# microsoft/fadtk

Measured on AMD Instinct MI355X. Metric: FAD scores/sec + cov-GEMM TFLOP/s (% MFMA peak), N=100k D=512, higher is better.
Workload: dtype f16 in, f16 MFMA with f32 accumulate over <= 8192-row runs, f64 across runs (moments); split-f16 MFMA iterations (f32 accumulate) + exact int8-MFMA products (int32 accumulate) + f64 correction (Frechet)

## Files before the change

### fadtk_amd/csrc/frechet.hip

```cpp
#include "frechet_internal.h"
#include "ns_mean.h"
#include "ns_fast.h"
#include "ns_fast_big.h"
#include "ns_fast_res.h"

#include <algorithm>
#include <atomic>
#include <cmath>
#include <type_traits>

namespace fad {

Pool& thread_pool(int device) {
    static thread_local PerThreadDevice<Pool> set;
    return set.get(device);
}
Workspace* free_slot(int device) {
    Pool& p = thread_pool(device);
    for (Workspace& w : p.slot)
        if (!w.busy) { w.pool = &p; return &w; }
    return nullptr;
}

SongKnobs SongKnobs::from_env() {
// ... 582 lines not shown
    int k = 1, upto = resident ? 1 : 9;
    for (;;) {
        for (; k < upto; ++k) {
            const int cur = k & 1;
            nsf::SplitArgs g = split_args();
            g.A[0] = Z[cur]; g.B[0] = Y[cur]; g.C[0] = T; g.alpha = -0.5f; g.beta_eye = 1.5f; g.gamma = 1.0f;
            g.partials = partials; g.skip = &s32_0->done; g.k = k;
            if (big) FAD_TRY(fast_split_big(d, nsf::SP_T, g, st, (unsigned)B, device));
            else fast_split(d, nsf::SP_T, g, st, (unsigned)B);
            g = split_args();
            g.A[0] = Y[cur]; g.B[0] = T; g.C[0] = Y[cur ^ 1]; g.A[1] = T; g.B[1] = Z[cur]; g.C[1] = Z[cur ^ 1];
            g.skip = &s32_0->upd_skip[k & 1];
            g.k = k; g.max_low = kMaxLow; g.nslots = big ? fast_big_t_slots(d, (unsigned)B) : nb * nb; g.chk_partials = partials; g.thr_pred = pred_threshold(ws.pool, d);
            if (big) FAD_TRY(fast_split_big(d, nsf::SP_U, g, st, (unsigned)B, device));
            else fast_split(d, nsf::SP_U, g, st, (unsigned)B);
        }
        if (!res_full) {
            nsf::DigArgs dg;
            memset(&dg, 0, sizeof(dg));
            dg.d = d; dg.gen = gen; dg.hA = hdr_b; dg.hB = reinterpret_cast<nsf::MatHdr*>(at(L.hdr)); dg.pstride = (int64_t)L.stride; dg.s32 = s32_0;
            dg.Y[0] = Y[0]; dg.Y[1] = Y[1]; dg.dig[0] = digY[0]; dg.dig[1] = digY[1]; dg.dig_t[0] = digYt[0]; dg.dig_t[1] = digYt[1];
            hipLaunchKernelGGL(nsf::nsf_digitize, dim3((unsigned)((dd / 16 + 255) / 256), 2, (unsigned)B), dim3(256), 0, st, dg);
        }
        if (!res_full) {
            nsf::I8Args a;
            memset(&a, 0, sizeof(a));
            a.Adig = digY[0]; a.Bdig = digYt[0]; a.Adig_alt = digY[1]; a.Bdig_alt = digYt[1]; a.sel = &s32_0->final_iter;
            a.d = d; a.gen = gen; a.hA = hdr_b; a.hB = reinterpret_cast<nsf::MatHdr*>(at(L.hdr)); a.pstride = (int64_t)L.stride; a.hstride = (int64_t)hs;
            a.skip = &s32_0->skip_corr; a.stats = h_stats; a.st = st0; a.A64in = A64;
            a.Y[0] = Y[0]; a.Y[1] = Y[1]; a.Z[0] = Z[0]; a.Z[1] = Z[1]; a.s32 = s32_0; a.host_words = h_words; a.host_vals = h_vals;
            for (int64_t b = 0; b < B; ++b) reinterpret_cast<int*>(reinterpret_cast<char*>(h_words) + b * hs)[12] = 0;
            if (big && d >= 256) FAD_TRY(fast_i8_big(d, nsf::I8_G, a, st, (unsigned)B, device));
            else fast_i8(d, nsf::I8_G, a, st, (unsigned)B);
        }
        FAD_HIP_TRY(hipGetLastError());
        FAD_HIP_TRY(hipStreamSynchronize(st));
        bool pending = false;
        for (int64_t b = 0; b < B; ++b) {
            if (settled[b]) continue;
            const int* hw = reinterpret_cast<const int*>(reinterpret_cast<const char*>(h_words) + b * hs);
            const double* hv = reinterpret_cast<const double*>(reinterpret_cast<const char*>(h_vals) + b * hs);
            const double* hx = reinterpret_cast<const double*>(reinterpret_cast<const char*>(h_stats) + b * hs);
            if (hw[12] != gen) return set_error(FAD_ERR_HIP, "the correction kernel of the batched fast chain left no result for song %lld", (long long)b);
            MixedResult r;
            fast_decide_one(hw, hv, hx, nb, &r);
            if (r.status == 0 && k < kMaxLow && !resident) { pending = true; continue; }
            settled[b] = 1;
            if (r.status == 1) { ok[b] = 1; tr_sqrt[b] = std::sqrt(r.c) * r.tr_scaled; }
            if (trace)
                fprintf(stderr, "[fad fast songs] song %lld: status %d iters %d decided_at %d res %.3e est %.3e tr %.6e c %.3e (words bad %d done %d ok %d failed %d skipped %d)\n",
                        (long long)b, r.status, r.iters, r.decided_at, r.res, r.est, r.tr_scaled, r.c, hw[0], hw[1], hw[5], hw[6], hw[11]);
            if (trace && b == 0) {
                fprintf(stderr, "[fad fast songs] song 0 residuals:");
                for (int q = 1; q < 16 && q <= r.iters; ++q) fprintf(stderr, " %.3e", hv[4 + q]);
                fprintf(stderr, "\n");
            }
        }
        if (!pending) break;
        upto = kMaxLow;
    }
    return FAD_OK;
}


struct PairBlock {
    size_t hdrA, hdrB, st, s32, partials, stats, A64, P, Y[2], Z[2], T, digA, digB, digY[2], digYt[2], mus, covs, Rv, Pv, Ev, stride;
};
static PairBlock pair_block(int d) {
    const size_t dd = (size_t)d * d, nb = (size_t)d / 32;
    PairBlock b; size_t o = 0;
    auto take = [&](size_t bytes) { const size_t at = o; o += (bytes + 255) & ~(size_t)255; return at; };
    b.hdrA = take(sizeof(nsf::MatHdr)); b.hdrB = take(sizeof(nsf::MatHdr)); b.st = take(sizeof(NsState)); b.s32 = take(sizeof(Ns32State));
    b.partials = take(nb * nb * sizeof(double)); b.stats = take(nsf::kTileStats * nb * nb * sizeof(double));
    b.A64 = take(8 * dd); b.P = take(8 * dd);
    b.Y[0] = take(8 * dd); b.Y[1] = take(8 * dd); b.Z[0] = take(8 * dd); b.Z[1] = take(8 * dd); b.T = take(8 * dd);
    b.digA = take(6 * dd); b.digB = take(6 * dd);
    b.digY[0] = take(6 * dd); b.digYt[0] = take(6 * dd); b.digY[1] = take(6 * dd); b.digYt[1] = take(6 * dd);
    b.mus = take(2 * (size_t)d * sizeof(double)); b.covs = take(2 * dd * sizeof(double));
    b.Rv = take(8 * dd); b.Pv = take(8 * dd); b.Ev = take(8 * dd);
    b.stride = o;
    return b;
}

static int pairs_verify_enqueue(Workspace& ws, int d, int B, hipStream_t st) {
    const size_t dd = (size_t)d * d;
    const PairBlock L = pair_block(d);
    const size_t hs = song_host_stride(d);
    char* blk = static_cast<char*>(ws.fast_pairs.p);
    char* hpin = static_cast<char*>(ws.fast_pairs_pin);
    auto at = [&](size_t off) { return blk + off; };
    auto mat = [&](size_t off) { nsf::SplitMat m; m.a = reinterpret_cast<uint4*>(at(off)); m.at = reinterpret_cast<uint4*>(at(off + 4 * dd)); return m; };
    nsf::SplitArgs g;
    memset(&g, 0, sizeof(g));
    g.d = d; g.gen = ws.multi.gen; g.hA = reinterpret_cast<nsf::MatHdr*>(at(L.hdrA)); g.hB = reinterpret_cast<nsf::MatHdr*>(at(L.hdrB));
    g.pstride = (int64_t)L.stride; g.astride = (int64_t)L.stride;
    g.st = reinterpret_cast<NsState*>(at(L.st)); g.s32 = reinterpret_cast<Ns32State*>(at(L.s32));
    const nsf::SplitMat Y[2] = {mat(L.Y[0]), mat(L.Y[1])}, Z[2] = {mat(L.Z[0]), mat(L.Z[1])};
    const int nb = d / 32;
    int* h_words = reinterpret_cast<int*>(hpin + (nsf::kHostVals + (size_t)(nsf::kTileStats + 2) * nb * nb) * sizeof(double));
    double* h_vstats = reinterpret_cast<double*>(hpin + host_vstats_off(d));
    for (int b = 0; b < B; ++b) reinterpret_cast<int*>(reinterpret_cast<char*>(h_words) + (size_t)b * hs)[13] = 0;
    fast_verify_launch(d, (unsigned)B, g, Y, Z, mat(L.Rv), mat(L.Pv), mat(L.Ev), g.s32, h_vstats, h_words, (int64_t)hs, st);
    FAD_HIP_TRY(hipGetLastError());
    FAD_HIP_TRY(hipEventRecord(ws.done_ev, st));
    return FAD_OK;
}

static int pairs_enqueue(Workspace& ws, int d, int B, const fad_moments_t* const* h1, const fad_moments_t* const* h2, int ddof,
                         int mean_dtype, hipStream_t st) {
    const size_t dd = (size_t)d * d;
    const int nb = d / 32;
    constexpr int kPairsBigMin = 3;
    const bool big = B >= kPairsBigMin && d >= 256;
    const bool wide = wide_enabled(ws.pool);
    const int max_low = wide ? kMaxLowWide : kMaxLow;
    const int device = ws.job.device;
    const PairBlock L = pair_block(d);
    const size_t hs = song_host_stride(d);
    void* const before = ws.fast_pairs.p;
    FAD_TRY(ws.fast_pairs.reserve((size_t)(B > 16 ? kMaxMultiPairs : B > 8 ? 16 : B > 4 ? 8 : 4) * L.stride + 256));
    if (!ws.fast_pairs_pin || ws.fast_pairs_pin_cap < (size_t)B * hs) {
        if (ws.fast_pairs_pin) (void)hipHostFree(ws.fast_pairs_pin);
        ws.fast_pairs_pin = nullptr; ws.fast_pairs_pin_cap = 0;
        FAD_HIP_TRY(hipHostMalloc(&ws.fast_pairs_pin, (size_t)kMaxMultiPairs * hs + 4096, hipHostMallocDefault));
        ws.fast_pairs_pin_cap = (size_t)kMaxMultiPairs * hs + 4096;
    }
    char* blk = static_cast<char*>(ws.fast_pairs.p);
    char* hpin = static_cast<char*>(ws.fast_pairs_pin);
    double* h_vals = reinterpret_cast<double*>(hpin);
    double* h_stats = h_vals + nsf::kHostVals;
    int* h_words = reinterpret_cast<int*>(h_stats + (size_t)(nsf::kTileStats + 2) * nb * nb);
    auto at = [&](size_t off) { return blk + off; };
    auto mat = [&](size_t off) { nsf::SplitMat m; m.a = reinterpret_cast<uint4*>(at(off)); m.at = reinterpret_cast<uint4*>(at(off + 4 * dd)); return m; };
    const int gen = ++ws.fast_gen;
    if (ws.fast_gen > (1 << 30)) ws.fast_gen = 1;
    ws.multi.gen = gen;
    if (ws.fast_pairs.p != before) {
        FAD_HIP_TRY(hipMemset2DAsync(at(L.hdrA), L.stride, 0, sizeof(nsf::MatHdr), (size_t)B, st));
        FAD_HIP_TRY(hipMemset2DAsync(at(L.hdrB), L.stride, 0, sizeof(nsf::MatHdr), (size_t)B, st));
    }
    nsf::MatHdr* hA = reinterpret_cast<nsf::MatHdr*>(at(L.hdrA));
    nsf::MatHdr* hB = reinterpret_cast<nsf::MatHdr*>(at(L.hdrB));
    NsState* st0 = reinterpret_cast<NsState*>(at(L.st));
    Ns32State* s32_0 = reinterpret_cast<Ns32State*>(at(L.s32));
    double* partials = reinterpret_cast<double*>(at(L.partials));
    double* stats = reinterpret_cast<double*>(at(L.stats));
    double* A64 = reinterpret_cast<double*>(at(L.A64));
    const nsf::SplitMat P = mat(L.P), Y[2] = {mat(L.Y[0]), mat(L.Y[1])}, Z[2] = {mat(L.Z[0]), mat(L.Z[1])}, T = mat(L.T);
    uint4* digY[2] = {reinterpret_cast<uint4*>(at(L.digY[0])), reinterpret_cast<uint4*>(at(L.digY[1]))};
    uint4* digYt[2] = {reinterpret_cast<uint4*>(at(L.digYt[0])), reinterpret_cast<uint4*>(at(L.digYt[1]))};

    static_assert(2 * kMaxMultiPairs <= nsf::kPrepMaxSets, "PrepArgs holds two sets per pair of a batch");
    nsf::PrepArgs pa;
    memset(&pa, 0, sizeof(pa));
    for (int b = 0; b < B; ++b) {
        pa.accs[2 * b] = moments_packed(h1[b]); pa.accs[2 * b + 1] = moments_packed(h2[b]);
        pa.runs[2 * b] = moments_runsum(h1[b]); pa.runs[2 * b + 1] = moments_runsum(h2[b]);
    }
    pa.acc[0] = pa.accs[0]; pa.acc[1] = pa.accs[1];
    pa.d = d; pa.ddof = ddof; pa.gen = gen; pa.mean_dtype = mean_dtype;
    pa.mus = reinterpret_cast<double*>(at(L.mus)); pa.covs = reinterpret_cast<double*>(at(L.covs));
    pa.dig[0] = reinterpret_cast<uint4*>(at(L.digA)); pa.dig[1] = reinterpret_cast<uint4*>(at(L.digB));
    pa.st = st0; pa.hdr[0] = hA; pa.hdr[1] = hB;
    pa.batch = 2; pa.pstride = (int64_t)L.stride; pa.no_covs = 1;
    pa.per = ((dd / 2048) % 4 == 0) ? 4 : 2;
    hipLaunchKernelGGL(nsf::nsf_prepare, dim3((unsigned)(dd / 2048 / pa.per + 1), (unsigned)(2 * B)), dim3(512), 0, st, pa);

    auto split_args = [&]() {
        nsf::SplitArgs g;
        memset(&g, 0, sizeof(g));
        g.d = d; g.gen = gen; g.hA = hA; g.hB = hB; g.pstride = (int64_t)L.stride; g.astride = (int64_t)L.stride;
        g.st = st0; g.s32 = s32_0;
        if (wide) { g.scaled = 1; g.lp_wide = 1; g.l0_scale = kWideL0Scale; g.l0_min = kWideL0Min; }
        return g;
    };
    {
        nsf::I8Args a;
        memset(&a, 0, sizeof(a));
        a.Adig = reinterpret_cast<uint4*>(at(L.digA)); a.Bdig = reinterpret_cast<uint4*>(at(L.digB)); a.d = d; a.gen = gen; a.hA = hA; a.hB = hB;
        a.pstride = (int64_t)L.stride; a.astride = (int64_t)L.stride; a.stats = stats; a.A64 = A64; a.P = P; a.st = st0;
        if (big) FAD_TRY(fast_i8_big(d, nsf::I8_A, a, st, (unsigned)B, device));
        else fast_i8(d, nsf::I8_A, a, st, (unsigned)B);
        nsf::SplitArgs g = split_args();
        g.A[0] = P; g.B[0] = P; g.C[0] = Y[1]; g.C[1] = Z[1]; g.A64 = A64; g.statsA = stats;
        if (big) FAD_TRY(fast_split_big(d, nsf::SP_FIRST, g, st, (unsigned)B, device));
        else { g.Cdig[0] = digY[1]; g.Cdig_t[0] = digYt[1]; fast_split(d, nsf::SP_FIRST, g, st, (unsigned)B); }
    }
    int want = ws.pool ? ws.pool->lp_iters : 5;
    if (want < 2) want = 2;
    if (want > max_low) want = max_low;
    for (int k = 1; k < want; ++k) {
        const int cur = k & 1;
        nsf::SplitArgs g = split_args();
        g.A[0] = Z[cur]; g.B[0] = Y[cur]; g.C[0] = T; g.alpha = -0.5f; g.beta_eye = 1.5f; g.gamma = 1.0f;
        g.partials = partials; g.skip = &s32_0->done; g.k = k;
        if (big) FAD_TRY(fast_split_big(d, nsf::SP_T, g, st, (unsigned)B, device));
        else fast_split(d, nsf::SP_T, g, st, (unsigned)B);
        g = split_args();
        g.A[0] = Y[cur]; g.B[0] = T; g.C[0] = Y[cur ^ 1]; g.A[1] = T; g.B[1] = Z[cur]; g.C[1] = Z[cur ^ 1];
        if (!big) { g.Cdig[0] = digY[cur ^ 1]; g.Cdig_t[0] = digYt[cur ^ 1]; }
        g.skip = &s32_0->upd_skip[k & 1];
        g.k = k; g.max_low = max_low; g.nslots = big ? fast_big_t_slots(d, (unsigned)B) : nb * nb; g.chk_partials = partials; g.thr_pred = pred_threshold(ws.pool, d);
        if (big) FAD_TRY(fast_split_big(d, nsf::SP_U, g, st, (unsigned)B, device));
        else fast_split(d, nsf::SP_U, g, st, (unsigned)B);
    }
    if (big) {
        nsf::DigArgs dg;
        memset(&dg, 0, sizeof(dg));
        dg.d = d; dg.gen = gen; dg.hA = hA; dg.hB = hB; dg.pstride = (int64_t)L.stride; dg.astride = (int64_t)L.stride; dg.s32 = s32_0;
        dg.Y[0] = Y[0]; dg.Y[1] = Y[1]; dg.dig[0] = digY[0]; dg.dig[1] = digY[1]; dg.dig_t[0] = digYt[0]; dg.dig_t[1] = digYt[1];
        hipLaunchKernelGGL(nsf::nsf_digitize, dim3((unsigned)((dd / 16 + 255) / 256), 2, (unsigned)B), dim3(256), 0, st, dg);
    }
    {
        nsf::I8Args a;
        memset(&a, 0, sizeof(a));
        a.Adig = digY[0]; a.Bdig = digYt[0]; a.Adig_alt = digY[1]; a.Bdig_alt = digYt[1]; a.sel = &s32_0->final_iter;
        a.d = d; a.gen = gen; a.hA = hA; a.hB = hB; a.pstride = (int64_t)L.stride; a.astride = (int64_t)L.stride; a.hstride = (int64_t)hs;
        a.skip = &s32_0->skip_corr; a.stats = h_stats; a.st = st0; a.A64in = A64;
        a.Y[0] = Y[0]; a.Y[1] = Y[1]; a.Z[0] = Z[0]; a.Z[1] = Z[1]; a.s32 = s32_0; a.host_words = h_words; a.host_vals = h_vals;
        if (wide) { a.Rv = mat(L.Rv); a.scaled = 1; }
        for (int b = 0; b < B; ++b) { int* w = reinterpret_cast<int*>(reinterpret_cast<char*>(h_words) + (size_t)b * hs); w[12] = 0; w[13] = 0; }
        if (big) FAD_TRY(fast_i8_big(d, nsf::I8_G, a, st, (unsigned)B, device));
        else fast_i8(d, nsf::I8_G, a, st, (unsigned)B);
    }
    FAD_HIP_TRY(hipGetLastError());
    if (!ws.done_ev) FAD_HIP_TRY(hipEventCreateWithFlags(&ws.done_ev, hipEventDisableTiming));
    if (wide && ws.pool && ws.pool->lp_verify) return pairs_verify_enqueue(ws, d, B, st);
    FAD_HIP_TRY(hipEventRecord(ws.done_ev, st));
    return FAD_OK;
}

static int mixed_begin(const NsProblem& pb, int device, hipStream_t stream, Workspace& ws) {
    const int d = pb.d;
    const int64_t dd = (int64_t)d * d;
    FAD_TRY(ws.mats.reserve((size_t)(6 * dd) * sizeof(double)));
    FAD_TRY(ws.mats32.reserve((size_t)(5 * dd) * sizeof(float)));
    const size_t hbytes = ws.job.fast ? fast_pinned_bytes(d) : sizeof(NsState) + sizeof(MixedResult);
    if (!ws.pinned || ws.pinned_cap < hbytes) {
        if (ws.pinned) (void)hipHostFree(ws.pinned);
        ws.pinned = nullptr; ws.pinned_cap = 0;
        FAD_HIP_TRY(hipHostMalloc(&ws.pinned, hbytes + 4096, hipHostMallocDefault));
        ws.pinned_cap = hbytes + 4096;
    }
    MixedBufs m = mixed_bufs(ws, d);
    m.hres->status = -1;
    ws.job.d = d; ws.job.device = device; ws.job.stream = stream; ws.job.k = 0;
    if (ws.job.fast) {
        ws.job.mu1 = pb.mu1; ws.job.mu2 = pb.mu2; ws.job.mean_dtype = pb.mean_dtype;
        int want = ws.pool ? ws.pool->lp_iters : 5;
        if (want < 2) want = 2;
        if (want > max_low_of(ws)) want = max_low_of(ws);
        if (ws.pool && ws.pool->lp_hopeless) want = 1;
        return fast_enqueue(ws, want);
    }
    NsProductExt ext;
    memset(&ext, 0, sizeof(ext));
    ext.stats = m.tilestats; ext.mu1 = pb.mu1; ext.mu2 = pb.mu2; ext.mean_dtype = pb.mean_dtype; ext.st = m.dstate;
    FAD_TRY(gemm_f64_product_stats_launch(d, pb.cov1, pb.cov2, m.A, &m.dstate->done, ext, stream));
    enqueue_ns_prepare(m.tilestats, d, (int)m.nb, pb.mu1, 0, pb.mu2, 0, pb.mean_dtype, m.dstate, 1, m.s32, 1, stream);
    int want = ws.pool ? ws.pool->lp_iters : 5;
    if (want < 2) want = 2;
    if (want > kMaxLow) want = kMaxLow;
    return mixed_enqueue(ws, want);
}

static int mixed_finish(Workspace& ws, MixedResult* res) {
    MixedBufs m = mixed_bufs(ws, ws.job.d);
    const int max_low = max_low_of(ws);
    bool asked = false;
    for (;;) {
        FAD_HIP_TRY(hipEventSynchronize(ws.done_ev));
        if (ws.job.fast) FAD_TRY(fast_decide(ws));
        if (m.hres->status == 5) {
            if (asked) { m.hres->status = 2; break; }
            asked = true;
            FAD_TRY(fast_verify_enqueue(ws));
            continue;
        }
        if (m.hres->status == 4) {
            ws.job.k = m.hres->iters;
            m.hres->status = 0;
        } else if (m.hres->status != 0 || ws.job.k >= max_low) {
            break;
        }
        if (ws.job.k >= max_low) break;
        const int step = (ws.job.fast && max_low > kMaxLow) ? 4 : 2;
        const int upto = (ws.job.k + step < max_low) ? ws.job.k + step : max_low;
        FAD_TRY(ws.job.fast ? fast_enqueue(ws, upto) : mixed_enqueue(ws, upto));
    }
    *res = *m.hres;
    if (res->status == 0) res->status = 2;
    if (res->status == 1 && res->decided_at >= 0 && ws.pool) ws.pool->lp_iters = res->decided_at + 1;
    if (ws.pool && ws.job.fast) {
        ws.pool->lp_hopeless = res->status == 2 && res->iters < 0;
        ws.pool->lp_verify = res->status == 1 && res->pad == 1;
    }
    return FAD_OK;
}

static bool mixed_eligible(Workspace& ws, int d, int max_iter, double tol) {
    Pool* p = ws.pool;
    if (p && p->mixed < 0) { const char* e = getenv("FAD_FRECHET_MIXED"); p->mixed = (e && e[0] == '0') ? 0 : 1; }
    return (!p || p->mixed) && d % 64 == 0 && max_iter <= 0 && tol <= 0.0;
}

static int frechet_single(int d, const double* cov1, const double* cov2, const double* mu1, const double* mu2,
                          double eps, int max_iter, double tol, int mean_dtype, int device, hipStream_t stream,
                          Workspace& ws, double* out_fad, fad_diag_t* diag, bool check_few) {
    const int64_t dd = (int64_t)d * d;
    NsState* hs = nullptr;
// ... 348 lines not shown
```

### fadtk_amd/csrc/frechet_internal.h

```cpp
#pragma once
#include "fad_common.h"
#include "ns_check.h"
#include "ns32.h"

#include <cstdlib>
#include <vector>

struct fad_moments;
namespace fad {
const double* moments_packed(const fad_moments* h);
int moments_settle(const fad_moments* h, hipStream_t st);
int moments_mark_read(const fad_moments* h, hipStream_t st);
int moments_device(const fad_moments* h);
int moments_dim(const fad_moments* h);
const float* moments_runsum(const fad_moments* h);

constexpr int kStatScal = 8;
static inline int64_t stat_blocks(int d) { return cdiv(d, 32); }
static inline size_t stat_doubles(int d) { const int64_t nb = stat_blocks(d); return (size_t)(2 * nb * d + kStatScal * nb * nb); }

constexpr int kMaxMultiPairs = 32;

struct Workspace : NsWorkspace {
    DevBuf rows, offs, songbuf, songmat, rows2, songrun, songjobs;
    DevBuf base_root;
    void* song_pin = nullptr; size_t song_pin_cap = 0;
    DevBuf mats32;
    DevBuf fast;
    int fast_gen = 0;
    DevBuf songcov;
    DevBuf fast_songs;
    void* fast_songs_pin = nullptr; size_t fast_songs_pin_cap = 0;
    DevBuf fast_pairs;
    void* fast_pairs_pin = nullptr; size_t fast_pairs_pin_cap = 0;
    struct Multi {
        int count = 0, gen = 0;
        bool enqueued = false;
        const fad_moments_t* h1[kMaxMultiPairs] = {nullptr}; const fad_moments_t* h2[kMaxMultiPairs] = {nullptr};
    } multi;
    bool busy = false;
    struct Job {
        int d = 0, device = 0, k = 0, mean_dtype = -1, ddof = 1;
        bool mixed = false;
        bool fast = false;
        int gen = 0;
        double eps = 0.0;
        hipStream_t stream = nullptr;
        const double *cov1 = nullptr, *cov2 = nullptr, *mu1 = nullptr, *mu2 = nullptr;
    } job;
    hipEvent_t done_ev = nullptr;
    struct Pool* pool = nullptr;
    void release_all() {
        release(); rows.release(); offs.release(); songbuf.release(); songmat.release(); rows2.release(); songrun.release(); songjobs.release(); mats32.release(); base_root.release(); fast.release();
        fast_songs.release(); songcov.release(); fast_pairs.release();
        if (fast_pairs_pin) { (void)hipHostFree(fast_pairs_pin); fast_pairs_pin = nullptr; fast_pairs_pin_cap = 0; }
        if (fast_songs_pin) { (void)hipHostFree(fast_songs_pin); fast_songs_pin = nullptr; fast_songs_pin_cap = 0; }
        if (done_ev) { (void)hipEventDestroy(done_ev); done_ev = nullptr; }
        if (song_pin) { (void)hipHostFree(song_pin); song_pin = nullptr; song_pin_cap = 0; }
    }
    int reserve_song_pin(size_t bytes) {
        if (song_pin && song_pin_cap >= bytes) return FAD_OK;
        if (song_pin) (void)hipHostFree(song_pin);
        song_pin = nullptr; song_pin_cap = 0;
        FAD_HIP_TRY(hipHostMalloc(&song_pin, bytes + bytes / 2 + 4096, hipHostMallocDefault));
        song_pin_cap = bytes + bytes / 2 + 4096;
        return FAD_OK;
    }
};


struct Pool {
    static constexpr int kSlots = 8;
    Workspace slot[kSlots];
    int lp_iters = 5;
    bool lp_hopeless = false;
    bool lp_verify = false;
    int lp_wide = -1;
    int f64_iters = 0;
    int f64_iters_multi = 0;
    int mixed = -1;
    int fast = -1;
    double pred_thr = 0.0;
    void release_all() { for (Workspace& w : slot) w.release_all(); }
};
Pool& thread_pool(int device);
Workspace* free_slot(int device);

struct NsProblem {
    int d; int64_t B;
    const double* cov1; int64_t s_cov1;
    const double* cov2; int64_t s_cov2;
    const double* mu1; int64_t s_mu1;
    const double* mu2; int64_t s_mu2;
    int mean_dtype;
    int sym = 0;
};

static inline int ns_pstride(int d) {
    const int64_t a = gemm_f64_slots_max(d), b = cdiv((int64_t)d * d, 256);
    return (int)(a > b ? a : b);
}
static inline size_t ns_small_bytes(int d, int64_t B) {
    return (size_t)B * (sizeof(NsState) + sizeof(Ns32State) + ((size_t)ns_pstride(d) + stat_doubles(d)) * sizeof(double)) + 256;
}

__device__ __forceinline__ void sum_partials(const double* __restrict__ rowabs, const double* __restrict__ colabs, int nb,
                                             int d, int i, double& rs, double& cs) {
    rs = 0.0; cs = 0.0;
    int k = 0;
    for (; k + 8 <= nb; k += 8) {
        double r[8], c[8];
#pragma unroll
        for (int q = 0; q < 8; ++q) { r[q] = rowabs[(int64_t)(k + q) * d + i]; c[q] = colabs[(int64_t)(k + q) * d + i]; }
#pragma unroll
        for (int q = 0; q < 8; ++q) { rs += r[q]; cs += c[q]; }
    }
    for (; k < nb; ++k) { rs += rowabs[(int64_t)k * d + i]; cs += colabs[(int64_t)k * d + i]; }
}

constexpr int kSymMaxIter = 16;

int run_ns(const NsProblem& pb, int max_iter, double tol, int device, hipStream_t stream, Workspace& ws,
           NsState** host_states, bool reuse_prepared = false, double** y_bufs = nullptr, int first_chunk = 0);
void enqueue_mark_states_done(NsState* st, uint32_t mask, int B, hipStream_t stream);
void enqueue_clear_states(NsState* st, int64_t B, hipStream_t stream);
void enqueue_add_diag(double* M, int d, double eps, hipStream_t stream);
void enqueue_finalize_for_frechet(const double* acc1, const double* acc2, int d, int ddof, double* mus, double* covs, NsState* st,
                                  hipStream_t stream, const float* run1 = nullptr, const float* run2 = nullptr);
void enqueue_ns_prepare(const double* stats_all, int d, int nb, const double* mu1, int64_t m1, const double* mu2, int64_t m2,
                        int mean_dtype, NsState* st_all, int mean_given, Ns32State* s32, int64_t B, hipStream_t stream);

bool fast_song_dim(int d);
int64_t fast_songs_capacity(int d, size_t budget_bytes);
struct SongKnobs {
    long big_min = 8;
    int res = 2;
    int fast = 1;
    bool trace = false;
    double l0_scale = 0.5;
    bool scaled = true;
    static SongKnobs from_env();
};
int fast_songs(int d, int64_t B, const double* dcov_b, const double* covs, hipStream_t st, Workspace& ws,
               std::vector<double>& tr_sqrt, std::vector<char>& ok, int device, const SongKnobs& knobs);

}
```

### fadtk_amd/csrc/ns_fast_big.h

```cpp
#pragma once
#include "ns_fast.h"
#include "big_slots.h"

namespace fad {
namespace nsf {

#ifndef FAD_BIG_STAGES
#define FAD_BIG_STAGES 3
#endif
constexpr int kBigStages = FAD_BIG_STAGES;
constexpr int kBigStage = 1024;
constexpr size_t kBigLds = (size_t)kBigStages * kBigStage * 16 + 256;

template <int MODE, int NJ = 2>
__global__ __launch_bounds__(256, (FAD_BIG_STAGES <= 3) ? 3 : ((FAD_BIG_STAGES <= 4) ? 2 : 1)) void nsf_big(SplitArgs g) {
    static_assert(MODE == SP_T || MODE == SP_U || MODE == SP_FIRST, "SP_FIRST: iteration 0 (scale from nsf_i8<A>'s statistics, Y1, Z1)");
    extern __shared__ __attribute__((aligned(16))) uint4 ring[];
    double* red = reinterpret_cast<double*>(ring + kBigStages * kBigStage);
    const int d = g.d, tid = threadIdx.x, lane = tid & 63;
    constexpr int ZP = (MODE == SP_U) ? 2 : 1;
    const int t = d >> 7, tx_n = (NJ == 2) ? t : 2 * t, tt = t * tx_n;
    const int L = blockIdx.x;
    const int nprod = big_grid(g.nprob, tt * ZP);
    if constexpr (MODE == SP_U) {
// ... 215 lines not shown
    if constexpr (MODE == SP_T) {
        double s1[1] = {ss};
        wg8_sum<1, 4>(s1, red);
        if (tid == 0) adv(g.partials, po)[tile] = s1[0];
    }
}

constexpr int kI8BigStage = 36 * 64;
#ifndef FAD_I8_BIG_STAGES
#define FAD_I8_BIG_STAGES 2
#endif
constexpr int kI8BigStages = FAD_I8_BIG_STAGES;
constexpr size_t kI8BigLds = (size_t)kI8BigStages * kI8BigStage * 16 + 256;

template <int MODE, bool WITHR = false>
__global__ __launch_bounds__(512) void nsf_i8_big(I8Args g, int nprob) {
    extern __shared__ __attribute__((aligned(16))) uint4 ring[];
    double* red = reinterpret_cast<double*>(ring + kI8BigStages * kI8BigStage);
    constexpr int kUmin = (MODE == I8_A) ? kUminA : kUminG;
    constexpr int kGroups = 2 * (kDigits - 1) - kUmin + 1;
    const int d = g.d, tid = threadIdx.x, lane = tid & 63;
    const int tr_ = d >> 7, tc_ = d >> 6, tt = tr_ * tc_;
    const BigSlot slot = big_slot(blockIdx.x, nprob, tt);
    if (!slot.live) return;
    const int song = slot.song, tile = slot.item;
    const int TY = tile / tc_, TX = tile - TY * tc_;
    const int64_t po = (int64_t)song * g.pstride, ho = (int64_t)song * g.hstride;
    const MatHdr* hB = adv(g.hB, po);
    const MatHdr* hA = adv(g.hA, (int64_t)song * g.astride);
    NsState* const st_p = adv(g.st, po);
    const bool bad = hdr_bad(hA, hB, g.gen);
    const bool skipped = bad || (g.skip && *adv(g.skip, po) != 0);
    if constexpr (MODE == I8_G) {
        if (tile == 0 && tid == 0) {
            const NsState* st = st_p; const Ns32State* s = adv(g.s32, po);
            int* hw = adv(g.host_words, ho); double* hv = adv(g.host_vals, ho);
            hw[0] = bad ? 1 : 0; hw[1] = st->done; hw[2] = st->nonfinite; hw[3] = st->too_few[0]; hw[4] = st->too_few[1];
            hw[5] = s->ok; hw[6] = s->failed; hw[7] = s->final_iter; hw[8] = s->decided_at; hw[9] = s->strict; hw[10] = s->finished;
            hw[11] = skipped ? 1 : 0;
            hv[0] = st->c; hv[1] = st->tr1; hv[2] = st->tr2; hv[3] = st->mean_term;
#pragma unroll
            for (int q = 0; q < 16; ++q) hv[4 + q] = s->res[q];
            hw[14] = (g.scaled && st->mu[0] != 1.0) ? 1 : 0;
            hw[12] = g.gen;
        }
    }
    if (skipped) return;
    const int wave = __builtin_amdgcn_readfirstlane(tid >> 6);
    const int wr = wave >> 1, wc = wave & 1;
    const bool alt = (MODE == I8_G) && g.sel && (*adv(g.sel, po) & 1);
    const uint4* Ad = (MODE == I8_A) ? adv(g.Adig, (int64_t)song * g.astride) : adv(alt ? g.Adig_alt : g.Adig, po);
    const uint4* Bd = adv(alt ? g.Bdig_alt : g.Bdig, po);
#ifdef FAD_I8_ABL_G_NOLOOP
    const int nks = (MODE == I8_G) ? 0 : (d >> 5);
#else
    const int nks = d >> 5;
#endif

    const uint32_t voff = (uint32_t)lane * 16u;
    const uint32_t ring_lds = (uint32_t)(size_t)(__attribute__((address_space(3))) void*)ring;
    auto issue = [&](int ks) {
#pragma unroll
        for (int i = 0; i < 5; ++i) {
            const int q = wave + 8 * i;
            if (q < 36) {
                const bool bs = q >= 24;
                const int blk = bs ? (q - 24) / 6 : q / 6, p = bs ? (q - 24) % 6 : q % 6;
                const uint64_t sb = (uint64_t)((bs ? Bd : Ad) + dg_idx((bs ? 2 * TX : 4 * TY) + blk, ks, p, 0, d));
                const uint32_t lo = __builtin_amdgcn_readfirstlane((uint32_t)sb);
                const uint32_t hi = __builtin_amdgcn_readfirstlane((uint32_t)(sb >> 32));
                const uint64_t ub = ((uint64_t)hi << 32) | lo;
                const uint32_t m0v = __builtin_amdgcn_readfirstlane(ring_lds + (uint32_t)(((ks % kI8BigStages) * kI8BigStage + q * 64) * 16));
                asm volatile("s_mov_b32 m0, %2\n\ts_nop 0\n\tglobal_load_lds_dwordx4 %0, %1" ::"v"(voff), "s"(ub), "s"(m0v) : "memory", "m0");
            }
        }
    };
    i32x16 acc[kGroups];
#pragma unroll
    for (int u = 0; u < kGroups; ++u)
#pragma unroll
        for (int q = 0; q < 16; ++q) acc[u][q] = 0;
    static_assert(kI8BigStages >= 2 && kI8BigStages <= 4, "the counted waits below cover two younger stages at most");
    for (int ks = 0; ks < kI8BigStages - 1 && ks < nks; ++ks) issue(ks);
    const bool five = wave < 4;
    for (int ks = 0; ks < nks; ++ks) {
        const int ahead = (nks - 1 - ks < kI8BigStages - 2) ? (nks - 1 - ks) : (kI8BigStages - 2);
        if (ahead == 2) { if (five) asm volatile("s_waitcnt vmcnt(10)" ::: "memory"); else asm volatile("s_waitcnt vmcnt(8)" ::: "memory"); }
        else if (ahead == 1) { if (five) asm volatile("s_waitcnt vmcnt(5)" ::: "memory"); else asm volatile("s_waitcnt vmcnt(4)" ::: "memory"); }
        else asm volatile("s_waitcnt vmcnt(0)" ::: "memory");
        __builtin_amdgcn_s_barrier();
#ifndef FAD_I8_ABL_NODMA
        if (ks + kI8BigStages - 1 < nks) issue(ks + kI8BigStages - 1);
#endif
        const i32x4* st = reinterpret_cast<const i32x4*>(ring + (ks % kI8BigStages) * kI8BigStage) + lane;
        i32x4 a[kDigits], b[kDigits];
#pragma unroll
        for (int p = 0; p < kDigits; ++p) { a[p] = st[(wr * 6 + p) * 64]; b[p] = st[(24 + wc * 6 + p) * 64]; }
#ifdef FAD_I8_ABL_NOMMA
#pragma unroll
        for (int p = 0; p < kDigits; ++p) { acc[0][p] += a[p][0] ^ b[p][1]; acc[1][p] += a[p][2] ^ b[p][3]; }
#else
#pragma unroll
        for (int p = kDigits - 1; p >= 0; --p)
#pragma unroll
            for (int q = kDigits - 1; q >= 0; --q)
                if (p + q >= kUmin) acc[p + q - kUmin] = __builtin_amdgcn_mfma_i32_32x32x32_i8(a[p], b[q], acc[p + q - kUmin], 0, 0, 0);
#endif
    }
    __syncthreads();
    double gp[16];
#pragma unroll
    for (int q = 0; q < 16; ++q) gp[q] = 0.0;
#pragma unroll
    for (int u = 0; u < kGroups; ++u) {
        const double wgt = __builtin_ldexp(1.0, 7 * (u + kUmin) - 80);
#pragma unroll
        for (int q = 0; q < 16; ++q) gp[q] = __builtin_fma((double)acc[u][q], wgt, gp[q]);
    }
    float* fin = reinterpret_cast<float*>(ring) + wave * (32 * 33 + 32);
    const int kg = lane >> 5, n = lane & 31;
    const int by = 4 * TY + wr, bx = 2 * TX + wc, nb = d >> 5;
    const int row0 = 32 * by, col0 = 32 * bx;
    double* const stats = adv(g.stats, (MODE == I8_A) ? po : ho);
    double* scal = stats + (size_t)kTileStats * (by * nb + bx);
    double v3[3] = {0.0, 0.0, 0.0};
    if constexpr (MODE == I8_A) {
        const double inv = hdr_inv_s12(hA, hB);
        double* A64 = adv(g.A64, po) + (int64_t)(row0 + 4 * kg) * d + col0 + n;
#pragma unroll
        for (int reg = 0; reg < 16; ++reg) {
            const int q = (reg & 3) + 8 * (reg >> 2);
            A64[(int64_t)q * d] = gp[reg] * inv;
            fin[(q + 4 * kg) * 33 + n] = (float)gp[reg];
            v3[0] += gp[reg] * gp[reg];
            if (by == bx && q + 4 * kg == n) v3[1] += gp[reg];
        }
        __builtin_amdgcn_wave_barrier();
        const SplitMat Pm = adv(g.P, po);
#pragma unroll
        for (int pass = 0; pass < 4; ++pass) store_tile_planes(fin, Pm, by, bx, d, pass * 64 + lane);
    } else {
        const SplitMat Zm = adv(g.Z[alt ? 1 : 0], po);
        const SplitMat Ym = adv(g.Y[alt ? 1 : 0], po);
        const double inv_c = 1.0 / st_p->c;
        const double* A64 = adv(g.A64in, po) + (int64_t)(row0 + 4 * kg) * d + col0 + n;
        typedef _Float16 f16x4 __attribute__((ext_vector_type(4)));
        f16x4 zh[4], zl[4];
#pragma unroll
        for (int j = 0; j < 4; ++j) {
            int half;
            const size_t zi = fa_elem(col0 + n, row0 + 8 * j + 4 * kg, 0, d, half);
            zh[j] = *reinterpret_cast<const f16x4*>(reinterpret_cast<const _Float16*>(Zm.a + zi) + half);
            zl[j] = *reinterpret_cast<const f16x4*>(reinterpret_cast<const _Float16*>(Zm.a + zi + 64) + half);
        }
#pragma unroll
        for (int reg = 0; reg < 16; ++reg) {
            const int q = (reg & 3) + 8 * (reg >> 2), gr = row0 + q + 4 * kg, gc = col0 + n;
            const double R = A64[(int64_t)q * d] * inv_c - gp[reg];
            if constexpr (WITHR) gp[reg] = R;
            const double z = (double)used16(zh[reg >> 2][reg & 3], zl[reg >> 2][reg & 3]);
            v3[0] += z * R; v3[1] += R * R;
            if (by == bx && gr == gc) {
                int hy;
                const size_t yi = fa_elem(gr, gr, 0, d, hy);
                v3[2] += (double)used16(reinterpret_cast<const _Float16*>(Ym.a + yi)[hy], reinterpret_cast<const _Float16*>(Ym.a + yi + 64)[hy]);
            }
            fin[(q + 4 * kg) * 33 + n] = fabsf((float)z);
        }
        __builtin_amdgcn_wave_barrier();
    }
    double m = 0.0;
    if constexpr (MODE == I8_A) {
        if (lane < 32) { for (int c = 0; c < 32; ++c) m += fabsf(fin[lane * 33 + c]); }
        else { for (int q = 0; q < 32; ++q) m += fabsf(fin[q * 33 + lane - 32]); }
    } else {
        if (lane < 32) { for (int q = 0; q < 32; ++q) m += fin[q * 33 + lane]; }
        else { for (int c = 0; c < 32; ++c) m += fin[(lane - 32) * 33 + c]; }
    }
    double mrow = (lane < 32) ? m : 0.0, mcol = (lane >= 32) ? m : 0.0;
#pragma unroll
    for (int off = 32; off > 0; off >>= 1) {
        mrow = fmax(mrow, __shfl_xor(mrow, off)); mcol = fmax(mcol, __shfl_xor(mcol, off));
#pragma unroll
        for (int q = 0; q < 3; ++q) v3[q] += __shfl_xor(v3[q], off);
    }
    if (lane == 0) {
        if constexpr (MODE == I8_A) {
            scal[0] = v3[0]; scal[1] = v3[1]; scal[2] = mrow; scal[3] = mcol;
        } else {
            scal[0] = v3[0]; scal[1] = v3[1]; scal[2] = v3[2]; scal[3] = 0.0;
            double* zmax = stats + (size_t)kTileStats * nb * nb + 2 * (size_t)(by * nb + bx);
            zmax[0] = mrow; zmax[1] = mcol;
        }
    }
    if constexpr (MODE == I8_G && WITHR) {
        if (g.Rv.a) {
            __builtin_amdgcn_wave_barrier();
#pragma unroll
            for (int reg = 0; reg < 16; ++reg) fin[((reg & 3) + 8 * (reg >> 2) + 4 * kg) * 33 + n] = (float)(gp[reg] * (double)kVerScale);
            __builtin_amdgcn_wave_barrier();
            const SplitMat Rm = adv(g.Rv, po);
#pragma unroll
            for (int pass = 0; pass < 4; ++pass) store_tile_planes(fin, Rm, by, bx, d, pass * 64 + lane);
        }
    }
    (void)red;
}

}
}
```

Baseline: 12010.

## Split pair batches across two streams and prefetch epilogue operands before K loop

Batched Frechet pair processing is refactored into a range-based enqueue. When FAD_CHAIN_LANES=2, the second half of the batch runs on a separate lane stream forked after the first I8_A stage and joined with events, so the two halves' Newton-Schulz chains can overlap. Separately, the big int8 kernel now loads the A64 residual values, the Z planes and the Y diagonal before the main MFMA loop, so that latency hides behind the matrix work instead of stalling the epilogue. This costs extra registers, and the stream split is opt-in, disabled during graph capture, and adds stream/event bookkeeping.

```diff
diff --git a/fadtk_amd/csrc/frechet.hip b/fadtk_amd/csrc/frechet.hip
--- a/fadtk_amd/csrc/frechet.hip
+++ b/fadtk_amd/csrc/frechet.hip
@@ -688,12 +688,12 @@
     return b;
 }
 
-static int pairs_verify_enqueue(Workspace& ws, int d, int B, hipStream_t st) {
+static int pairs_verify_range(Workspace& ws, int d, int b0, int n, hipStream_t st) {
     const size_t dd = (size_t)d * d;
     const PairBlock L = pair_block(d);
     const size_t hs = song_host_stride(d);
-    char* blk = static_cast<char*>(ws.fast_pairs.p);
-    char* hpin = static_cast<char*>(ws.fast_pairs_pin);
+    char* blk = static_cast<char*>(ws.fast_pairs.p) + (size_t)b0 * L.stride;
+    char* hpin = static_cast<char*>(ws.fast_pairs_pin) + (size_t)b0 * hs;
     auto at = [&](size_t off) { return blk + off; };
     auto mat = [&](size_t off) { nsf::SplitMat m; m.a = reinterpret_cast<uint4*>(at(off)); m.at = reinterpret_cast<uint4*>(at(off + 4 * dd)); return m; };
     nsf::SplitArgs g;
@@ -705,46 +705,36 @@
     const int nb = d / 32;
     int* h_words = reinterpret_cast<int*>(hpin + (nsf::kHostVals + (size_t)(nsf::kTileStats + 2) * nb * nb) * sizeof(double));
     double* h_vstats = reinterpret_cast<double*>(hpin + host_vstats_off(d));
-    for (int b = 0; b < B; ++b) reinterpret_cast<int*>(reinterpret_cast<char*>(h_words) + (size_t)b * hs)[13] = 0;
-    fast_verify_launch(d, (unsigned)B, g, Y, Z, mat(L.Rv), mat(L.Pv), mat(L.Ev), g.s32, h_vstats, h_words, (int64_t)hs, st);
+    for (int b = 0; b < n; ++b) reinterpret_cast<int*>(reinterpret_cast<char*>(h_words) + (size_t)b * hs)[13] = 0;
+    fast_verify_launch(d, (unsigned)n, g, Y, Z, mat(L.Rv), mat(L.Pv), mat(L.Ev), g.s32, h_vstats, h_words, (int64_t)hs, st);
     FAD_HIP_TRY(hipGetLastError());
+    return FAD_OK;
+}
+static int pairs_verify_enqueue(Workspace& ws, int d, int B, hipStream_t st) {
+    FAD_TRY(pairs_verify_range(ws, d, 0, B, st));
     FAD_HIP_TRY(hipEventRecord(ws.done_ev, st));
     return FAD_OK;
 }
 
-static int pairs_enqueue(Workspace& ws, int d, int B, const fad_moments_t* const* h1, const fad_moments_t* const* h2, int ddof,
-                         int mean_dtype, hipStream_t st) {
+constexpr int kPairsBigMin = 3;
+
+static int pairs_enqueue_range(Workspace& ws, int d, int b0, int n, const fad_moments_t* const* h1, const fad_moments_t* const* h2, int ddof,
+                               int mean_dtype, int gen, hipStream_t st, hipEvent_t after_a) {
     const size_t dd = (size_t)d * d;
     const int nb = d / 32;
-    constexpr int kPairsBigMin = 3;
-    const bool big = B >= kPairsBigMin && d >= 256;
+    const bool big = n >= kPairsBigMin && d >= 256;
     const bool wide = wide_enabled(ws.pool);
     const int max_low = wide ? kMaxLowWide : kMaxLow;
     const int device = ws.job.device;
     const PairBlock L = pair_block(d);
     const size_t hs = song_host_stride(d);
-    void* const before = ws.fast_pairs.p;
-    FAD_TRY(ws.fast_pairs.reserve((size_t)(B > 16 ? kMaxMultiPairs : B > 8 ? 16 : B > 4 ? 8 : 4) * L.stride + 256));
-    if (!ws.fast_pairs_pin || ws.fast_pairs_pin_cap < (size_t)B * hs) {
-        if (ws.fast_pairs_pin) (void)hipHostFree(ws.fast_pairs_pin);
-        ws.fast_pairs_pin = nullptr; ws.fast_pairs_pin_cap = 0;
-        FAD_HIP_TRY(hipHostMalloc(&ws.fast_pairs_pin, (size_t)kMaxMultiPairs * hs + 4096, hipHostMallocDefault));
-        ws.fast_pairs_pin_cap = (size_t)kMaxMultiPairs * hs + 4096;
-    }
-    char* blk = static_cast<char*>(ws.fast_pairs.p);
-    char* hpin = static_cast<char*>(ws.fast_pairs_pin);
+    char* blk = static_cast<char*>(ws.fast_pairs.p) + (size_t)b0 * L.stride;
+    char* hpin = static_cast<char*>(ws.fast_pairs_pin) + (size_t)b0 * hs;
     double* h_vals = reinterpret_cast<double*>(hpin);
     double* h_stats = h_vals + nsf::kHostVals;
     int* h_words = reinterpret_cast<int*>(h_stats + (size_t)(nsf::kTileStats + 2) * nb * nb);
     auto at = [&](size_t off) { return blk + off; };
     auto mat = [&](size_t off) { nsf::SplitMat m; m.a = reinterpret_cast<uint4*>(at(off)); m.at = reinterpret_cast<uint4*>(at(off + 4 * dd)); return m; };
-    const int gen = ++ws.fast_gen;
-    if (ws.fast_gen > (1 << 30)) ws.fast_gen = 1;
-    ws.multi.gen = gen;
-    if (ws.fast_pairs.p != before) {
-        FAD_HIP_TRY(hipMemset2DAsync(at(L.hdrA), L.stride, 0, sizeof(nsf::MatHdr), (size_t)B, st));
-        FAD_HIP_TRY(hipMemset2DAsync(at(L.hdrB), L.stride, 0, sizeof(nsf::MatHdr), (size_t)B, st));
-    }
     nsf::MatHdr* hA = reinterpret_cast<nsf::MatHdr*>(at(L.hdrA));
     nsf::MatHdr* hB = reinterpret_cast<nsf::MatHdr*>(at(L.hdrB));
     NsState* st0 = reinterpret_cast<NsState*>(at(L.st));
@@ -759,9 +749,9 @@
     static_assert(2 * kMaxMultiPairs <= nsf::kPrepMaxSets, "PrepArgs holds two sets per pair of a batch");
     nsf::PrepArgs pa;
     memset(&pa, 0, sizeof(pa));
-    for (int b = 0; b < B; ++b) {
-        pa.accs[2 * b] = moments_packed(h1[b]); pa.accs[2 * b + 1] = moments_packed(h2[b]);
-        pa.runs[2 * b] = moments_runsum(h1[b]); pa.runs[2 * b + 1] = moments_runsum(h2[b]);
+    for (int b = 0; b < n; ++b) {
+        pa.accs[2 * b] = moments_packed(h1[b0 + b]); pa.accs[2 * b + 1] = moments_packed(h2[b0 + b]);
+        pa.runs[2 * b] = moments_runsum(h1[b0 + b]); pa.runs[2 * b + 1] = moments_runsum(h2[b0 + b]);
     }
     pa.acc[0] = pa.accs[0]; pa.acc[1] = pa.accs[1];
     pa.d = d; pa.ddof = ddof; pa.gen = gen; pa.mean_dtype = mean_dtype;
@@ -770,7 +760,7 @@
     pa.st = st0; pa.hdr[0] = hA; pa.hdr[1] = hB;
     pa.batch = 2; pa.pstride = (int64_t)L.stride; pa.no_covs = 1;
     pa.per = ((dd / 2048) % 4 == 0) ? 4 : 2;
-    hipLaunchKernelGGL(nsf::nsf_prepare, dim3((unsigned)(dd / 2048 / pa.per + 1), (unsigned)(2 * B)), dim3(512), 0, st, pa);
+    hipLaunchKernelGGL(nsf::nsf_prepare, dim3((unsigned)(dd / 2048 / pa.per + 1), (unsigned)(2 * n)), dim3(512), 0, st, pa);
 
     auto split_args = [&]() {
         nsf::SplitArgs g;
@@ -785,12 +775,13 @@
         memset(&a, 0, sizeof(a));
         a.Adig = reinterpret_cast<uint4*>(at(L.digA)); a.Bdig = reinterpret_cast<uint4*>(at(L.digB)); a.d = d; a.gen = gen; a.hA = hA; a.hB = hB;
         a.pstride = (int64_t)L.stride; a.astride = (int64_t)L.stride; a.stats = stats; a.A64 = A64; a.P = P; a.st = st0;
-        if (big) FAD_TRY(fast_i8_big(d, nsf::I8_A, a, st, (unsigned)B, device));
-        else fast_i8(d, nsf::I8_A, a, st, (unsigned)B);
+        if (big) FAD_TRY(fast_i8_big(d, nsf::I8_A, a, st, (unsigned)n, device));
+        else fast_i8(d, nsf::I8_A, a, st, (unsigned)n);
+        if (after_a) FAD_HIP_TRY(hipEventRecord(after_a, st));
         nsf::SplitArgs g = split_args();
         g.A[0] = P; g.B[0] = P; g.C[0] = Y[1]; g.C[1] = Z[1]; g.A64 = A64; g.statsA = stats;
-        if (big) FAD_TRY(fast_split_big(d, nsf::SP_FIRST, g, st, (unsigned)B, device));
-        else { g.Cdig[0] = digY[1]; g.Cdig_t[0] = digYt[1]; fast_split(d, nsf::SP_FIRST, g, st, (unsigned)B); }
+        if (big) FAD_TRY(fast_split_big(d, nsf::SP_FIRST, g, st, (unsigned)n, device));
+        else { g.Cdig[0] = digY[1]; g.Cdig_t[0] = digYt[1]; fast_split(d, nsf::SP_FIRST, g, st, (unsigned)n); }
     }
     int want = ws.pool ? ws.pool->lp_iters : 5;
     if (want < 2) want = 2;
@@ -800,22 +791,22 @@
         nsf::SplitArgs g = split_args();
         g.A[0] = Z[cur]; g.B[0] = Y[cur]; g.C[0] = T; g.alpha = -0.5f; g.beta_eye = 1.5f; g.gamma = 1.0f;
         g.partials = partials; g.skip = &s32_0->done; g.k = k;
-        if (big) FAD_TRY(fast_split_big(d, nsf::SP_T, g, st, (unsigned)B, device));
-        else fast_split(d, nsf::SP_T, g, st, (unsigned)B);
+        if (big) FAD_TRY(fast_split_big(d, nsf::SP_T, g, st, (unsigned)n, device));
+        else fast_split(d, nsf::SP_T, g, st, (unsigned)n);
         g = split_args();
         g.A[0] = Y[cur]; g.B[0] = T; g.C[0] = Y[cur ^ 1]; g.A[1] = T; g.B[1] = Z[cur]; g.C[1] = Z[cur ^ 1];
         if (!big) { g.Cdig[0] = digY[cur ^ 1]; g.Cdig_t[0] = digYt[cur ^ 1]; }
         g.skip = &s32_0->upd_skip[k & 1];
-        g.k = k; g.max_low = max_low; g.nslots = big ? fast_big_t_slots(d, (unsigned)B) : nb * nb; g.chk_partials = partials; g.thr_pred = pred_threshold(ws.pool, d);
-        if (big) FAD_TRY(fast_split_big(d, nsf::SP_U, g, st, (unsigned)B, device));
-        else fast_split(d, nsf::SP_U, g, st, (unsigned)B);
+        g.k = k; g.max_low = max_low; g.nslots = big ? fast_big_t_slots(d, (unsigned)n) : nb * nb; g.chk_partials = partials; g.thr_pred = pred_threshold(ws.pool, d);
+        if (big) FAD_TRY(fast_split_big(d, nsf::SP_U, g, st, (unsigned)n, device));
+        else fast_split(d, nsf::SP_U, g, st, (unsigned)n);
     }
     if (big) {
         nsf::DigArgs dg;
         memset(&dg, 0, sizeof(dg));
         dg.d = d; dg.gen = gen; dg.hA = hA; dg.hB = hB; dg.pstride = (int64_t)L.stride; dg.astride = (int64_t)L.stride; dg.s32 = s32_0;
         dg.Y[0] = Y[0]; dg.Y[1] = Y[1]; dg.dig[0] = digY[0]; dg.dig[1] = digY[1]; dg.dig_t[0] = digYt[0]; dg.dig_t[1] = digYt[1];
-        hipLaunchKernelGGL(nsf::nsf_digitize, dim3((unsigned)((dd / 16 + 255) / 256), 2, (unsigned)B), dim3(256), 0, st, dg);
+        hipLaunchKernelGGL(nsf::nsf_digitize, dim3((unsigned)((dd / 16 + 255) / 256), 2, (unsigned)n), dim3(256), 0, st, dg);
     }
     {
         nsf::I8Args a;
@@ -825,13 +816,64 @@
         a.skip = &s32_0->skip_corr; a.stats = h_stats; a.st = st0; a.A64in = A64;
         a.Y[0] = Y[0]; a.Y[1] = Y[1]; a.Z[0] = Z[0]; a.Z[1] = Z[1]; a.s32 = s32_0; a.host_words = h_words; a.host_vals = h_vals;
         if (wide) { a.Rv = mat(L.Rv); a.scaled = 1; }
-        for (int b = 0; b < B; ++b) { int* w = reinterpret_cast<int*>(reinterpret_cast<char*>(h_words) + (size_t)b * hs); w[12] = 0; w[13] = 0; }
-        if (big) FAD_TRY(fast_i8_big(d, nsf::I8_G, a, st, (unsigned)B, device));
-        else fast_i8(d, nsf::I8_G, a, st, (unsigned)B);
+        for (int b = 0; b < n; ++b) { int* w = reinterpret_cast<int*>(reinterpret_cast<char*>(h_words) + (size_t)b * hs); w[12] = 0; w[13] = 0; }
+        if (big) FAD_TRY(fast_i8_big(d, nsf::I8_G, a, st, (unsigned)n, device));
+        else fast_i8(d, nsf::I8_G, a, st, (unsigned)n);
     }
     FAD_HIP_TRY(hipGetLastError());
+    if (wide && ws.pool && ws.pool->lp_verify) return pairs_verify_range(ws, d, b0, n, st);
+    return FAD_OK;
+}
+
+static int chain_lanes() { const char* e = getenv("FAD_CHAIN_LANES"); return (e && e[0] == '2') ? 2 : 1; }
+
+static int lane_cut(int B) {
+    const int mid = (B + 1) / 2, r8 = (mid + 4) & ~7;
+    return (r8 > 0 && r8 < B && 2 * r8 - B <= 4 && B - 2 * r8 <= 4) ? r8 : mid;
+}
+
+static int pairs_enqueue(Workspace& ws, int d, int B, const fad_moments_t* const* h1, const fad_moments_t* const* h2, int ddof,
+                         int mean_dtype, hipStream_t st) {
+    const PairBlock L = pair_block(d);
+    const size_t hs = song_host_stride(d);
+    void* const before = ws.fast_pairs.p;
+    FAD_TRY(ws.fast_pairs.reserve((size_t)(B > 16 ? kMaxMultiPairs : B > 8 ? 16 : B > 4 ? 8 : 4) * L.stride + 256));
+    if (!ws.fast_pairs_pin || ws.fast_pairs_pin_cap < (size_t)B * hs) {
+        if (ws.fast_pairs_pin) (void)hipHostFree(ws.fast_pairs_pin);
+        ws.fast_pairs_pin = nullptr; ws.fast_pairs_pin_cap = 0;
+        FAD_HIP_TRY(hipHostMalloc(&ws.fast_pairs_pin, (size_t)kMaxMultiPairs * hs + 4096, hipHostMallocDefault));
+        ws.fast_pairs_pin_cap = (size_t)kMaxMultiPairs * hs + 4096;
+    }
+    char* blk = static_cast<char*>(ws.fast_pairs.p);
+    const int gen = ++ws.fast_gen;
+    if (ws.fast_gen > (1 << 30)) ws.fast_gen = 1;
+    ws.multi.gen = gen;
+    if (ws.fast_pairs.p != before) {
+        FAD_HIP_TRY(hipMemset2DAsync(blk + L.hdrA, L.stride, 0, sizeof(nsf::MatHdr), (size_t)B, st));
+        FAD_HIP_TRY(hipMemset2DAsync(blk + L.hdrB, L.stride, 0, sizeof(nsf::MatHdr), (size_t)B, st));
+    }
     if (!ws.done_ev) FAD_HIP_TRY(hipEventCreateWithFlags(&ws.done_ev, hipEventDisableTiming));
-    if (wide && ws.pool && ws.pool->lp_verify) return pairs_verify_enqueue(ws, d, B, st);
+    Pool* const pool = ws.pool;
+    bool lanes = pool && B >= 2 * kPairsBigMin && d >= 256 && chain_lanes() == 2;
+    if (lanes) {
+        hipStreamCaptureStatus cs = hipStreamCaptureStatusNone;
+        if (hipStreamIsCapturing(st, &cs) != hipSuccess) { (void)hipGetLastError(); lanes = false; }
+        else if (cs != hipStreamCaptureStatusNone) lanes = false;
+    }
+    if (!lanes) {
+        FAD_TRY(pairs_enqueue_range(ws, d, 0, B, h1, h2, ddof, mean_dtype, gen, st, nullptr));
+        FAD_HIP_TRY(hipEventRecord(ws.done_ev, st));
+        return FAD_OK;
+    }
+    if (!pool->lane_stream) FAD_HIP_TRY(hipStreamCreateWithFlags(&pool->lane_stream, hipStreamNonBlocking));
+    if (!pool->lane_fork_ev) FAD_HIP_TRY(hipEventCreateWithFlags(&pool->lane_fork_ev, hipEventDisableTiming));
+    if (!pool->lane_join_ev) FAD_HIP_TRY(hipEventCreateWithFlags(&pool->lane_join_ev, hipEventDisableTiming));
+    const int cut = lane_cut(B);
+    FAD_TRY(pairs_enqueue_range(ws, d, 0, cut, h1, h2, ddof, mean_dtype, gen, st, pool->lane_fork_ev));
+    FAD_HIP_TRY(hipStreamWaitEvent(pool->lane_stream, pool->lane_fork_ev, 0));
+    FAD_TRY(pairs_enqueue_range(ws, d, cut, B - cut, h1, h2, ddof, mean_dtype, gen, pool->lane_stream, nullptr));
+    FAD_HIP_TRY(hipEventRecord(pool->lane_join_ev, pool->lane_stream));
+    FAD_HIP_TRY(hipStreamWaitEvent(st, pool->lane_join_ev, 0));
     FAD_HIP_TRY(hipEventRecord(ws.done_ev, st));
     return FAD_OK;
 }
diff --git a/fadtk_amd/csrc/frechet_internal.h b/fadtk_amd/csrc/frechet_internal.h
--- a/fadtk_amd/csrc/frechet_internal.h
+++ b/fadtk_amd/csrc/frechet_internal.h
@@ -81,7 +81,14 @@
     int mixed = -1;
     int fast = -1;
     double pred_thr = 0.0;
-    void release_all() { for (Workspace& w : slot) w.release_all(); }
+    hipStream_t lane_stream = nullptr;
+    hipEvent_t lane_fork_ev = nullptr, lane_join_ev = nullptr;
+    void release_all() {
+        for (Workspace& w : slot) w.release_all();
+        if (lane_fork_ev) { (void)hipEventDestroy(lane_fork_ev); lane_fork_ev = nullptr; }
+        if (lane_join_ev) { (void)hipEventDestroy(lane_join_ev); lane_join_ev = nullptr; }
+        if (lane_stream) { (void)hipStreamDestroy(lane_stream); lane_stream = nullptr; }
+    }
 };
 Pool& thread_pool(int device);
 Workspace* free_slot(int device);
diff --git a/fadtk_amd/csrc/ns_fast_big.h b/fadtk_amd/csrc/ns_fast_big.h
--- a/fadtk_amd/csrc/ns_fast_big.h
+++ b/fadtk_amd/csrc/ns_fast_big.h
@@ -321,6 +321,35 @@
         for (int q = 0; q < 16; ++q) acc[u][q] = 0;
     static_assert(kI8BigStages >= 2 && kI8BigStages <= 4, "the counted waits below cover two younger stages at most");
     for (int ks = 0; ks < kI8BigStages - 1 && ks < nks; ++ks) issue(ks);
+    const int kg = lane >> 5, n = lane & 31;
+    const int by = 4 * TY + wr, bx = 2 * TX + wc, nb = d >> 5;
+    const int row0 = 32 * by, col0 = 32 * bx;
+    typedef _Float16 f16x4 __attribute__((ext_vector_type(4)));
+    double pre_scale, a64[16], ydiag = 0.0;
+    f16x4 zh[4], zl[4];
+    if constexpr (MODE == I8_A) {
+        pre_scale = hdr_inv_s12(hA, hB);
+    } else {
+        const SplitMat Zm = adv(g.Z[alt ? 1 : 0], po);
+        const SplitMat Ym = adv(g.Y[alt ? 1 : 0], po);
+        pre_scale = 1.0 / st_p->c;
+        const double* A64 = adv(g.A64in, po) + (int64_t)(row0 + 4 * kg) * d + col0 + n;
+#pragma unroll
+        for (int reg = 0; reg < 16; ++reg) a64[reg] = A64[(int64_t)((reg & 3) + 8 * (reg >> 2)) * d];
+#pragma unroll
+        for (int j = 0; j < 4; ++j) {
+            int half;
+            const size_t zi = fa_elem(col0 + n, row0 + 8 * j + 4 * kg, 0, d, half);
+            zh[j] = *reinterpret_cast<const f16x4*>(reinterpret_cast<const _Float16*>(Zm.a + zi) + half);
+            zl[j] = *reinterpret_cast<const f16x4*>(reinterpret_cast<const _Float16*>(Zm.a + zi + 64) + half);
+        }
+        const int qd = n - 4 * kg;
+        if (by == bx && qd >= 0 && (qd & 4) == 0) {
+            int hy;
+            const size_t yi = fa_elem(row0 + n, row0 + n, 0, d, hy);
+            ydiag = (double)used16(reinterpret_cast<const _Float16*>(Ym.a + yi)[hy], reinterpret_cast<const _Float16*>(Ym.a + yi + 64)[hy]);
+        }
+    }
     const bool five = wave < 4;
     for (int ks = 0; ks < nks; ++ks) {
         const int ahead = (nks - 1 - ks < kI8BigStages - 2) ? (nks - 1 - ks) : (kI8BigStages - 2);
@@ -357,14 +386,11 @@
         for (int q = 0; q < 16; ++q) gp[q] = __builtin_fma((double)acc[u][q], wgt, gp[q]);
     }
     float* fin = reinterpret_cast<float*>(ring) + wave * (32 * 33 + 32);
-    const int kg = lane >> 5, n = lane & 31;
-    const int by = 4 * TY + wr, bx = 2 * TX + wc, nb = d >> 5;
-    const int row0 = 32 * by, col0 = 32 * bx;
     double* const stats = adv(g.stats, (MODE == I8_A) ? po : ho);
     double* scal = stats + (size_t)kTileStats * (by * nb + bx);
     double v3[3] = {0.0, 0.0, 0.0};
     if constexpr (MODE == I8_A) {
-        const double inv = hdr_inv_s12(hA, hB);
+        const double inv = pre_scale;
         double* A64 = adv(g.A64, po) + (int64_t)(row0 + 4 * kg) * d + col0 + n;
 #pragma unroll
         for (int reg = 0; reg < 16; ++reg) {
@@ -379,31 +405,15 @@
 #pragma unroll
         for (int pass = 0; pass < 4; ++pass) store_tile_planes(fin, Pm, by, bx, d, pass * 64 + lane);
     } else {
-        const SplitMat Zm = adv(g.Z[alt ? 1 : 0], po);
-        const SplitMat Ym = adv(g.Y[alt ? 1 : 0], po);
-        const double inv_c = 1.0 / st_p->c;
-        const double* A64 = adv(g.A64in, po) + (int64_t)(row0 + 4 * kg) * d + col0 + n;
-        typedef _Float16 f16x4 __attribute__((ext_vector_type(4)));
-        f16x4 zh[4], zl[4];
-#pragma unroll
-        for (int j = 0; j < 4; ++j) {
-            int half;
-            const size_t zi = fa_elem(col0 + n, row0 + 8 * j + 4 * kg, 0, d, half);
-            zh[j] = *reinterpret_cast<const f16x4*>(reinterpret_cast<const _Float16*>(Zm.a + zi) + half);
-            zl[j] = *reinterpret_cast<const f16x4*>(reinterpret_cast<const _Float16*>(Zm.a + zi + 64) + half);
-        }
+        const double inv_c = pre_scale;
 #pragma unroll
         for (int reg = 0; reg < 16; ++reg) {
             const int q = (reg & 3) + 8 * (reg >> 2), gr = row0 + q + 4 * kg, gc = col0 + n;
-            const double R = A64[(int64_t)q * d] * inv_c - gp[reg];
+            const double R = a64[reg] * inv_c - gp[reg];
             if constexpr (WITHR) gp[reg] = R;
             const double z = (double)used16(zh[reg >> 2][reg & 3], zl[reg >> 2][reg & 3]);
             v3[0] += z * R; v3[1] += R * R;
-            if (by == bx && gr == gc) {
-                int hy;
-                const size_t yi = fa_elem(gr, gr, 0, d, hy);
-                v3[2] += (double)used16(reinterpret_cast<const _Float16*>(Ym.a + yi)[hy], reinterpret_cast<const _Float16*>(Ym.a + yi + 64)[hy]);
-            }
+            if (by == bx && gr == gc) v3[2] += ydiag;
             fin[(q + 4 * kg) * 33 + n] = fabsf((float)z);
         }
         __builtin_amdgcn_wave_barrier();
```

After: 11870. -1.2%, worse.
